# hjurong/hand-pose-estimation

Measured on AMD Instinct MI355X. Metric: particle-evals/sec + tracked FPS, 320x240 depth, 256p x 30gen, higher is better.
Workload: dtype f32+f64

## Files before the change

hand-pose-estimation_amd/csrc/hpe_api.inc:

```
#include <chrono>
#include <cmath>
#include <cstdarg>
#include <cstdlib>
#include <cstdio>
#include <cstring>
#include <new>
#include <string>
#include <thread>
#include <vector>

#include <dlfcn.h>
#include <mutex>

#include <hip/hip_ext.h>
#include <rccl/rccl.h>

#include "../../include/hpe.h"
#include "hpe_host.hpp"

namespace {

#define HPE_RAW_RING 8

struct Slot {
// ... 278 lines not shown
    static constexpr int wpp2_max_p = 1024;
    bool fk_coop = true;
    bool use_graph = true;
    bool prep_split = true;
    double *h_pinned = nullptr;
    int *d_evals = nullptr;
    MwJob *d_mw_job = nullptr;
    double *d_mw_part = nullptr;
    unsigned *d_mw_ctr = nullptr;
    int *d_mw_err = nullptr;
    int *h_mw_err = nullptr, *h_mw_err_dev = nullptr;
    int mw_spin = MW_SPIN_MAX;
    int mw_fits = -1;
    bool refine_mw = true;
    bool refine_exact = false;
    unsigned long long captures = 0;
    int xch_every = 0;
    double *xch_ext = nullptr;
    hpe_exchange_fn xch_fn = nullptr;
    void *xch_user = nullptr;
    struct Subswarm {
        ncclComm_t comm = nullptr;
        double *d_script = nullptr;
        int *d_script_k = nullptr;
        int script_frames = 0;
        bool transport() const { return comm || d_script; }
        int nranks = 0, rank = 0;
        bool on = false;
        double *d_gath = nullptr;
        bool graphs = true;
// ... 615 lines not shown
        return HPE_E_HIP;
    }
    hpe::build_dev_hand(*hand, c->hand);
    if (dalloc(&c->d_hand, 1) != hipSuccess ||
        hipMemcpy(c->d_hand, &c->hand, sizeof(DevHand), hipMemcpyHostToDevice) != hipSuccess ||
        dalloc(&c->d_lane_hands, HPE_BATCH_MAX) != hipSuccess || reset_lane_hands(c) != hipSuccess ||
        dalloc(&c->d_state, 32) != hipSuccess || dalloc(&c->d_evals, 4) != hipSuccess ||
        hipMemset(c->d_evals, 0, 4 * sizeof(int)) != hipSuccess ||
        dalloc(&c->d_obs, HPE_MAX_SLOTS) != hipSuccess || dalloc(&c->d_obs_active, 1) != hipSuccess ||
        dalloc(&c->d_seq_obs, 1) != hipSuccess || dalloc(&c->d_seq_cur, 2) != hipSuccess ||
        dalloc(&c->d_mw_job, 1) != hipSuccess ||
        dalloc(&c->d_mw_part, (size_t)MW_MAX_Q * MW_MAX_NODES) != hipSuccess ||
        dalloc(&c->d_mw_ctr, MW_CTR_WORDS) != hipSuccess ||
        hipMemset(c->d_mw_ctr, 0, MW_CTR_WORDS * sizeof(unsigned)) != hipSuccess ||
        dalloc(&c->d_mw_err, 1) != hipSuccess || hipMemset(c->d_mw_err, 0, sizeof(int)) != hipSuccess ||
        hipHostMalloc((void **)&c->h_pinned, sizeof(double) * 256, 0) != hipSuccess ||
        hipHostMalloc((void **)&c->h_mw_err, sizeof(int), hipHostMallocMapped | hipHostMallocCoherent) != hipSuccess ||
        hipHostGetDevicePointer((void **)&c->h_mw_err_dev, c->h_mw_err, 0) != hipSuccess) {
        hpe_destroy(c);
        return HPE_E_HIP;
    }
    c->slots.resize(1);
    if (const char *pf = std::getenv("HPE_PSO_FORM"))
        c->pso_form = std::strcmp(pf, "block") == 0 ? 1 : std::strcmp(pf, "wave") == 0 ? 2 : 0;
    if (const char *wp = std::getenv("HPE_PSO_WPP")) {
        const int v = std::atoi(wp);
        c->pso_wpp = (v == 1 || v == 2) ? v : 0;
    }
    if (const char *fc = std::getenv("HPE_FK_COOP")) c->fk_coop = std::atoi(fc) != 0;
    if (const char *rm = std::getenv("HPE_REFINE_MW")) c->refine_mw = rm[0] != '0';
    if (const char *re = std::getenv("HPE_REFINE_EXACT")) c->refine_exact = re[0] == '1';
    if (const char *sp = std::getenv("HPE_MW_SPIN")) c->mw_spin = std::max(0, std::atoi(sp));
    if (const char *ps = std::getenv("HPE_PREP_SPLIT")) c->prep_split = ps[0] != '0';
    *c->h_mw_err = 0;
    const char *ng = std::getenv("HPE_NO_GRAPH");
    c->use_graph = !(ng && ng[0] == '1');
    *out = c;
    return HPE_OK;
}

static void drop_graphs(hpe_ctx *c) {
    if (c->stream) (void)hipStreamSynchronize(c->stream);
    for (GraphCache &gc : c->graphs) {
        for (auto &e : gc.entries) (void)hipGraphExecDestroy(e.exec);
        gc.entries.clear();
    }
}
// ... 23 lines not shown
    dfree(c->optl.d_obs);
    dfree(c->d_hand);
    dfree(c->d_lane_hands);
    dfree(c->d_theta);
    dfree(c->d_cost);
    dfree(c->d_terms);
    dfree(c->d_S);
    dfree(c->d_J);
    dfree(c->d_match);
    dfree(c->d_state);
    dfree(c->d_evals);
    dfree(c->d_mw_job);
    dfree(c->d_mw_part);
    dfree(c->d_mw_ctr);
    dfree(c->d_mw_err);
    dfree(c->d_render);
    dfree(c->d_obs);
    dfree(c->d_obs_active);
    dfree(c->d_seq_obs);
    dfree(c->d_seq_cur);
    dfree(c->d_bobs);
    dfree(c->d_bcur);
    dfree(c->d_bevals);
    for (auto &a : c->rb.arena) dfree(a);
    dfree(c->rb.d_obs);
    dfree(c->rb.d_info);
    dfree(c->rb.d_tab);
    dfree(c->rb.d_ctr);
    dfree(c->rb.d_raw);
    dfree(c->rb.d_cur);
// ... 516 lines not shown
#define RF_DYN_LDS (126u * 1024u)
static_assert(RF_DYN_LDS >= RF_STAGE_MAX * (3 * sizeof(double) + sizeof(int32_t)), "staging");

static bool mw_fits(hpe_ctx *c) {
    if (c->mw_fits < 0) {
        int per_cu = 0, cus = 0;
        auto k = c->refine_exact ? k_refine<false, true> : k_refine<false, true, true>;
        if (hipOccupancyMaxActiveBlocksPerMultiprocessor(&per_cu, k, RF_NT, prep_lds_bytes()) != hipSuccess ||
            hipDeviceGetAttribute(&cus, hipDeviceAttributeMultiprocessorCount, c->device) != hipSuccess)
            per_cu = cus = 0;
        c->mw_fits = (long)per_cu * cus >= 1 + MW_MAX_Q + PREP_WG ? 1 : 0;
    }
    return c->mw_fits == 1;
}

static int refine_launch(hpe_ctx *c, const FrameIo &io, int do_refine, const PrepArgs *pa = nullptr,
                         const PrepSplit *split = nullptr, DevPick *pick = nullptr) {
    int rc = ensure_match(c, (size_t)(io.n_max > 0 ? io.n_max : 1));
    if (rc) return rc;
    double *d_x0 = io.state;
    PrepArgs none;
    std::memset(&none, 0, sizeof(none));
    const PrepArgs a = pa ? *pa : none;
    const PrepSplit ps = (pa && split) ? *split : PrepSplit{};
    DevMw mw;
    std::memset(&mw, 0, sizeof(mw));
    const DevPick pk = pick ? *pick : DevPick{};
    if (pick) *pick = DevPick{};
    if (io.n_max <= RF_STAGE_MAX) {
        const dim3 grid(pa ? 1 + PREP_WG : 1);
        launch(c, HPE_PROF_REFINE, c->refine_exact ? k_refine<true> : k_refine<true, false, true>,
               grid, dim3(RF_NT), RF_DYN_LDS, d_x0, io.obs, (const DevHand *)c->d_hand,
               c->d_match, c->d_evals, do_refine, a, mw, pk, ps);
    } else if (c->refine_mw && mw_fits(c)) {
        mw.job = c->d_mw_job;
        mw.part = c->d_mw_part;
        mw.ctr = c->d_mw_ctr;
        mw.err = c->d_mw_err;
        mw.err_host = c->h_mw_err_dev;
        mw.Q = MW_MAX_Q;
        mw.spin = c->mw_spin;
        const dim3 grid(1 + MW_MAX_Q + (pa ? PREP_WG : 0));
        launch(c, HPE_PROF_REFINE,
               c->refine_exact ? k_refine<false, true> : k_refine<false, true, true>, grid,
               dim3(RF_NT), (unsigned)prep_lds_bytes(), d_x0, io.obs, (const DevHand *)c->d_hand,
               c->d_match, c->d_evals, do_refine, a, mw, pk, ps);
    } else {
        const dim3 grid(pa ? 1 + PREP_WG : 1);
        launch(c, HPE_PROF_REFINE, c->refine_exact ? k_refine<false> : k_refine<false, false, true>,
               grid, dim3(RF_NT), RF_DYN_LDS, d_x0,
               io.obs, (const DevHand *)c->d_hand, c->d_match, c->d_evals, do_refine, a,
               mw, pk, ps);
    }
    HIPCHK(c, hipGetLastError());
    return HPE_OK;
}

static int mw_check(hpe_ctx *c) {
    if (!c->d_mw_err) return HPE_OK;
    int err = 0;
    HIPCHK(c, hipMemcpy(&err, c->d_mw_err, sizeof(int), hipMemcpyDeviceToHost));
    if (!err && !(c->h_mw_err && *(volatile int *)c->h_mw_err)) return HPE_OK;
    HIPCHK(c, hipStreamSynchronize(c->stream));
    HIPCHK(c, hipMemset(c->d_mw_ctr, 0, MW_CTR_WORDS * sizeof(unsigned)));
    HIPCHK(c, hipMemset(c->d_mw_err, 0, sizeof(int)));
    if (c->h_mw_err) *(volatile int *)c->h_mw_err = 0;
    return fail(c, HPE_E_HIP, "multi-workgroup refine: a helper hand-off timed out (that "
// ... 208 lines not shown
    }
    if (gathered_out && set) {
        HIPCHK(c, hipSetDevice(c->device));
        HIPCHK(c, hipStreamSynchronize(c->stream));
        HIPCHK(c, hipMemcpy(gathered_out, c->ss.d_gath, sizeof(double) * c->ss.nranks * (HPE_DOF + 1),
                            hipMemcpyDeviceToHost));
    }
    return HPE_OK;
}

int hpe_set_refine_exact(hpe_ctx *c, int exact) {
    if (!c) return HPE_E_ARG;
    if (c->refine_exact != (exact != 0)) {
        c->refine_exact = exact != 0;
        c->mw_fits = -1;
        ++c->epoch;
    }
    return HPE_OK;
}

int hpe_get_refine_exact(const hpe_ctx *c) { return c && c->refine_exact ? 1 : 0; }

int hpe_graph_captures(const hpe_ctx *c, uint64_t *n) {
    if (!c || !n) return HPE_E_ARG;
    *n = c->captures;
    return HPE_OK;
}

int hpe_refine_init_pose(hpe_ctx *c, double x0[26], int32_t *evals_out) {
    if (!c) return HPE_E_ARG;
    if (!x0) return fail(c, HPE_E_ARG, "bad arguments");
    HIPCHK(c, hipSetDevice(c->device));
    DevObs o;
    int rc = need_frame(c, &o);
// ... 1558 lines not shown
```

hand-pose-estimation_amd/csrc/hpe_kernels.hip:

```cpp
#include <vector>

#include "hpe_device.hpp"
#include "hpe_prep.hpp"
#include "hpe_report.hpp"
#include "../../include/hpe.h"

__global__ __launch_bounds__(HPE_NT) void k_build(const double *__restrict__ theta, int P,
                                                  const DevHand *__restrict__ Hg,
                                                  double *__restrict__ S_out,
                                                  double *__restrict__ J_out) {
    __shared__ Smem sm;
    const int i = blockIdx.x, t = threadIdx.x;
    stage_hand<HPE_NT>(sm.hand, Hg);
    const DevHand *__restrict__ H = &sm.hand;
    if (t < HPE_DOF) sm.fk.th[t] = theta[(size_t)i * HPE_DOF + t];
    __syncthreads();
    if (t < 64) fk_wave(sm.fk, H);
    __syncthreads();
    if (t < 3 * HPE_NS) S_out[(size_t)i * 3 * HPE_NS + t] = (&sm.fk.S[0][0])[t];
    if (J_out && t < 63) {
        double v;
        if (t < 3) v = sm.fk.th[3 + t];
        else {
            const int row = t / 3, c = t % 3, k = (row - 1) / 4, jr = 1 + (row - 1) % 4;
// ... 786 lines not shown
            wave_sync();
            if (RIGID) rigid_wave<RG_ROT>(nodes[w], hq, thl);
            else fk_wave(nodes[w], H);
            const double al = wave_sum(align_frozen(nodes[w], cs, H, ms, l, 64));
            if (l == 0) mw.part[h * MW_MAX_NODES + w] = al;
        }
        asm volatile("s_waitcnt vmcnt(0)" ::: "memory");
        __syncthreads();
        if (t == 0) {
            __builtin_amdgcn_fence(__ATOMIC_RELEASE, "agent");
            atomicAdd(&mw.ctr[32 * (1 + h % MW_DONE_SHARDS)], 1u);
        }
    }
}

struct GoldShape {
    int n;
    unsigned long long nb;
    unsigned dn, up;
};
#define GOLD_BALANCED 0
#define GOLD_8 1
#define GOLD_4 2
#define GOLD_OPT8 3
#define GOLD_MIX 4
#ifndef HPE_GOLD_POLICY
#define HPE_GOLD_POLICY GOLD_MIX
#endif
template <int POL>
__device__ __forceinline__ GoldShape gold_shape(int ctx) {
// ... 5 lines not shown
    {8, 0x6043414240212000ull, 0xffff7531u, 0xfffff642u},
    {8, 0x6243414240212000ull, 0xfff7f531u, 0xfffff642u},
    {4, 0x0000000043212000ull, 0xfffffff1u, 0xfffff3f2u},
    {4, 0x0000000060402000ull, 0xfffff321u, 0xffffffffu},
    {4, 0x0000000040212000ull, 0xffffff31u, 0xfffffff2u},
    {8, 0xbf8f674340212000ull, 0xffffff31u, 0xf765f4f2u},
    {8, 0x6043414240212000ull, 0xffff7531u, 0xfffff642u},
    {8, 0x6743414240212000ull, 0xfffff531u, 0xf7fff642u},
    {8, 0xa080604340212000ull, 0xf76f5f31u, 0xfffff4f2u},
    {8, 0x6043414240212000ull, 0xffff7531u, 0xfffff642u},
    {4, 0x0000000040212000ull, 0xffffff31u, 0xfffffff2u},
    };
    return ctx == 0 ? T[3 * POL] : ctx == 1 ? T[3 * POL + 1] : T[3 * POL + 2];
}

template <bool MW = false, int POL = GOLD_BALANCED, bool UPD = false, bool RIGID = false, class CV>
__device__ __forceinline__ double gold_tree(RefineSm &rs, const DevObs &o, const CV &cv,
                                            const DevHand *__restrict__ H,
                                            const int32_t *__restrict__ match, double fk,
                                            double gp, double pl, double gl, int &evals,
                                            double *f_acc, FkX *Xt = nullptr,
                                            MwLeader *ml = nullptr, int *flag = nullptr,
                                            const FrozenPts *fp = nullptr, int rblk = 0,
                                            const double *md2p = nullptr) {
    const int t = threadIdx.x, w = t >> 6, l = t & 63;
    StampClock sc;
    sc.start();
    double A = 0, B = 1e100, alpha = 0.5, tk = 0;
    int it = 0, accepted = -1, ctx = 0;
    bool done = false;
    [[maybe_unused]] unsigned long long path = 0;
    while (!done) {
        const GoldShape sh = gold_shape<POL>(ctx);
        const int nn = sh.n;
        double thl = 0.0;
        if (w < nn) {
            const int nbw = (int)((sh.nb >> (8 * w)) & 0xff), len = nbw >> 5, bits = nbw & 31;
            double ga = A, gb = B, gal = alpha;
            for (int k = 0; k < len; ++k) {
                if ((bits >> k) & 1) gold_up(ga, gb, gal);
                else gold_down(ga, gb, gal);
            }
            thl = rs.x0[l < HPE_DOF ? l : 0] + gal * pl;
            if (l < HPE_DOF) rs.w[w].th[l] = thl;
        }
        eval_nodes<MW, RIGID>(rs, nn, o, cv, H, match, Xt, ml, flag, &thl, fp, rblk, md2p);
        if (MW && ml->failed) break;
        int node = 0;
        accepted = -1;
#pragma unroll
// ... 21 lines not shown
            } else {
                gold_down(A, B, alpha);
                node = (int)((sh.dn >> (4 * node)) & 15u);
                ctx = 1;
            }
        }
        if (!done && it >= 30) done = true;
        done = __builtin_amdgcn_readfirstlane(done ? 1 : 0) != 0;
        ctx = __builtin_amdgcn_readfirstlane(ctx);
        if (UPD && done && t < HPE_DOF) rs.x0[t] = rs.x0[t] - tk * gl;
        if (done && accepted >= 0) {
            for (int q = t; q < (int)(offsetof(FkSm, J) / 8); q += RF_NT)
                ((double *)&rs.base)[q] = ((const double *)&rs.w[accepted])[q];
            if (f_acc) *f_acc = rs.f[accepted];
        }
        __syncthreads();
        REF_TS(rs.ts_n, 4);
        sc.lap(19);
    }
    evals += it;
    if (HPE_STAMPS && blockIdx.x == 0 && t == 0) {
        hpe_stamps[9] += (tk != 0) ? 1 : 0;
        hpe_stamps[30] += (unsigned long long)it;
        hpe_stamps[32 + 9] += 1;
    }
#if HPE_STAMPS
    if (t == 0) {
        const unsigned long long k = atomicAdd(&hpe_gold_log[0], 1ull);
        if (k < HPE_GOLD_LOG)
            hpe_gold_log[1 + k] = path | ((unsigned long long)it << 32) |
                                  ((unsigned long long)(tk != 0) << 40);
    }
#endif
    return tk;
}

template <bool STAGED, bool MW = false, bool RIGID = false>
__global__ __launch_bounds__(RF_NT) void k_refine(double *__restrict__ x0g, const DevObs *__restrict__ og,
                                                  const DevHand *__restrict__ Hg,
                                                  int32_t *__restrict__ match_g,
                                                  int *__restrict__ evals_out, int do_refine,
                                                  PrepArgs pa, DevMw mw, DevPick pk, PrepSplit ps) {
    constexpr bool WIN = false;
    const DevWindow pw{};
#include "hpe_refine_body.inc"
}

enum LaneSrc { LANE_SRC_NONE, LANE_SRC_RAW, LANE_SRC_RING, LANE_SRC_U16 };
#define HPE_ACT_TRACK 1
#define HPE_ACT_PREP 2
__device__ __forceinline__ DevSwarm lane_swarm(DevSwarm sw, size_t stride) {
    const size_t off = stride * blockIdx.y;
    sw.xh = (double *)((char *)sw.xh + off);
    sw.pch = (double *)((char *)sw.pch + off);
    sw.pb = (double *)((char *)sw.pb + off);
    sw.v = (double *)((char *)sw.v + off);
    sw.inbox = (double *)((char *)sw.inbox + off);
    sw.gmin = (unsigned long long *)((char *)sw.gmin + off);
    sw.sig = (Sig *)((char *)sw.sig + off);
    sw.gpos = (double *)((char *)sw.gpos + off);
// ... 145 lines not shown
    const DevHand *__restrict__ const Hg = lane_hand<HANDS>(hands);
    double *__restrict__ const x0g = states + (size_t)HPE_STATE_N * blockIdx.y;
    const DevObs *__restrict__ const og = obs + blockIdx.y;
    int32_t *const match_g = nullptr;
    int *__restrict__ const evals_out = evals_b + HPE_EVALS_N * blockIdx.y;
    const int do_refine = SRC == LANE_SRC_NONE ? 1 : do_refine_arg;
    decltype(lane_prep<SRC>(tab, unit, raw_base, cur, 1)) pa{};
    DevWindow pw{};
    if (SRC != LANE_SRC_NONE && blockIdx.x >= 1) {
        pa = lane_prep<SRC>(tab, unit, raw_base, cur, 1);
        if (WIN) pw = wtab[blockIdx.y];
    }
    const DevMw mw{};
    const DevPick pk{};
    const PrepSplit ps{};
#include "hpe_refine_body.inc"
}
static_assert(PREP_NT == RF_NT, "the preparation workgroups ride in the refine launch");

struct WinPar {
    double margin_xy, margin_z, focal;
    int to_cm, pad;
};
__device__ __forceinline__ double wave_min_f64(double v) {
    for (int off = 32; off > 0; off >>= 1) v = fmin(v, __shfl_xor(v, off));
    return v;
}
__device__ __forceinline__ double wave_max_f64(double v) {
    for (int off = 32; off > 0; off >>= 1) v = fmax(v, __shfl_xor(v, off));
    return v;
// ... 292 lines not shown
```

hand-pose-estimation_amd/csrc/hpe_layout.hpp:

```cpp
#pragma once
#include <stdint.h>

#define HPE_NT 512
#define HPE_NW (HPE_NT / 64)
#define HPE_NS 48
#define HPE_MAX_SLOTS 4096
#define HPE_DOF 26
#define HPE_IMG_H 240
#define HPE_IMG_W 320

enum { ST_NORMAL = 1, ST_RP = 2, ST_RG = 3, ST_LINK = 4, ST_OPT_PERM = 5, ST_OPT_RP = 6,
       ST_OPT_RG = 7, ST_OPT_NORMAL = 8 };

struct DevHand {
    double Fc[5], Fs[5], FLc[5], FLs[5];
    double T10x[5], T10y[5];
    double L[5][4];
    double twc[5], tws[5];
    double radii[HPE_NS];
    double wa[HPE_NS], wb[HPE_NS];
    int32_t dg[HPE_NS], ja[HPE_NS];
};

struct DevObs {
// ... 74 lines not shown
    const double *gath;
    double *hist;
    const int *cur;
    int world;
};

struct DevMw {
    MwJob *job;
    double *part;
    unsigned *ctr;
    int *err;
    int *err_host;
    int Q;
    int spin;
};
```

hand-pose-estimation_amd/csrc/hpe_refine_body.inc:

```
    extern __shared__ __align__(16) unsigned char dyn[];
    const int nhelp = MW ? mw.Q : 0;
    if (MW && blockIdx.x >= 1 && (int)blockIdx.x <= nhelp) {
        if (do_refine) mw_helper<RIGID>(mw, blockIdx.x - 1, og, Hg, match_g);
        return;
    }
    if (blockIdx.x >= 1) {
        const unsigned long long t0 = HPE_STAMPS ? __builtin_amdgcn_s_memtime() : 0;
        prep_workgroup<WIN>(pa, blockIdx.x - 1 - nhelp, dyn, &ps, &pw);
        if (HPE_STAMPS && threadIdx.x == 0) {
            const int k = ((int)blockIdx.x - 1 - nhelp < PREP_BANDS) ? 24 : 25;
            atomicAdd(&hpe_stamps[k], __builtin_amdgcn_s_memtime() - t0);
            atomicAdd(&hpe_stamps[32 + k], 1ull);
        }
        return;
    }
    if (!do_refine) return;
    const DevObs o = *og;
    __shared__ RefineSm rs;
    __shared__ DevHand hs;
    const int t = threadIdx.x, w = t >> 6, l = t & 63;
    stage_hand<RF_NT>(hs, Hg);
    const DevHand *__restrict__ H = &hs;
    using CV = std::conditional_t<STAGED, CloudView, CloudGlobal>;
    CV cv;
    int32_t *match = match_g;
    if (STAGED) {
        double *cx = (double *)dyn, *cy = cx + o.n, *cz = cy + o.n;
        for (int p = t; p < o.n; p += RF_NT) {
            cx[p] = gp(o.cx)[p];
            cy[p] = gp(o.cy)[p];
            cz[p] = gp(o.cz)[p];
        }
        if constexpr (STAGED) cv = CV{cx, cy, cz, o.n};
        match = (int32_t *)(cz + o.n);
    }
    if constexpr (!STAGED) cv = obs_cloud(o);
    if (pk.gath) {
        if (w == 0) {
            const double x = pick_apply(pk.gath, pick_best_row(pk.gath, pk.world, l), l, x0g,
                                        pk.hist, pk.cur);
            if (l < HPE_DOF) rs.x0[l] = x;
        }
    } else if (t < HPE_DOF) {
        rs.x0[t] = x0g[t];
    }
    if (t == 0) rs.ts_n = 0;
    REF_TS(rs.ts_n, 0);
    __shared__ int mwflag;
    MwLeader ml{mw, 0u, false};
    __syncthreads();
    if (RIGID) {
        if (w == 0) {
            const double xl = rs.x0[l < HPE_DOF ? l : 0];
            const double thq = (l == 0) ? -180.0 : (l < 6) ? 0.0 : xl;
            if (l < HPE_DOF) rs.w[0].th[l] = thq;
            wave_sync();
            SphXYZ own;
            fk_wave<true>(rs.w[0], H, &own, &thq);
            if (l < HPE_NS) {
                rs.rg.q[l][0] = own.x;
                rs.rg.q[l][1] = own.y * -1;
                rs.rg.q[l][2] = own.z * -1;
            }
// ... 7 lines not shown
                co += (k < 2 || l < 16) ? v : 0.0;
            }
            co = wave_sum(co);
            if (l == 0) rs.rg.C = co;
        }
        __syncthreads();
    }
    StampClock sc;
    sc.start();
    int evals = 0;
    bool base_valid = false;
    const double e = 1e-5;
    const bool small = !MW && STAGED && o.n >= 1 && o.n <= FP_MAX;
    FrozenPts fpts;
    const double md2_l = depth_off_sq(o, H->radii[l < HPE_NS ? l : HPE_NS - 1]);
    for (int blk = 0; blk < 2; ++blk) {
        const int lo = 3 * blk;
        FkX *Xt = nullptr;
        if (RIGID && blk == 1) {
            if (w == 0) rigid_wave<RG_STORE_P>(rs.w[0], rs.rg, rs.x0[l < HPE_DOF ? l : 0], nullptr, rs.rg.P);
            __syncthreads();
        } else if (blk == 1) {
            if (w == 0) {
                if (l < HPE_DOF) rs.w[0].th[l] = rs.x0[l];
                wave_sync();
                fk_wave_t<FK_STORE_X, true>(rs.w[0], H, &rs.X);
            }
            __syncthreads();
            Xt = &rs.X;
        }
        double tol = 1;
        int cnt = 0, iter = 0;
        while (tol > 1e-6 && iter < 15 && cnt < 1 && !(MW && ml.failed)) {
            if (!base_valid) {
                if (t < HPE_DOF) rs.base.th[t] = rs.x0[t];
                __syncthreads();
                if (w == 0) {
                    if (RIGID) {
                        const double thl = rs.x0[l < HPE_DOF ? l : 0];
                        if (blk) rigid_wave<RG_TRANS>(rs.base, rs.rg, thl);
                        else rigid_wave<RG_ROT>(rs.base, rs.rg, thl);
                    } else if (Xt) {
                        fk_wave_t<FK_TRANSLATE>(rs.base, H, Xt);
                    } else {
                        fk_wave<true>(rs.base, H);
                    }
                }
                __syncthreads();
// ... 29 lines not shown
                double al;
                if (small) {
                    const bool spread = RIGID && HPE_RF_SPREAD;
                    const int f0 = (w < 4 || spread) ? 64 * w : (w >= 6) ? 256 + 128 * (w - 6) : 0;
                    const int cnt = (w < 4 || spread) ? 1 : (w >= 6) ? 2 : 0;
                    al = search_align<RF_NT, true>(rs.base, cv, H, match, load_pt(cv, f0 + l),
                                                   f0 + l, BT_GENS, 64, cnt);
                } else {
                    al = search_align<RF_NT, true>(rs.base, cv, H, match, load_pt(cv, t));
                }
                if (young) __builtin_amdgcn_s_setprio(0);
                double co = (!RIGID && t < 144) ? collide_term(rs.base, t, H) : 0.0;
                const double dep = depth_finish(dgc, o, t < HPE_NS);
                const double tot = wave_sum((al * o.lambda + dep) + co);
                if (l == 0) rs.red[w][0] = tot;
                head();
                __syncthreads();
                if (small) load_frozen_pts(fpts, cv, match, l);
                fk = 0;
#pragma unroll
                for (int k = 0; k < RF_NW; ++k) fk += rs.red[k][0];
                if (RIGID) fk = fk + rs.rg.C;
                REF_TS(rs.ts_n, 2);
                if (w < 6) {
                    double f = RIGID ? frozen_tail<true>(rs.w[w], o, cv, H, match, hd,
                                                         small ? &fpts : nullptr, &md2_l)
                                     : frozen_tail(rs.w[w], o, cv, H, match, hd, small ? &fpts : nullptr);
                    if (RIGID) f = f + rs.rg.C;
                    if (l == 0) rs.fg[w] = f;
                }
                __syncthreads();
            }
            ++evals;
            sc.lap(20);
            evals += 6;
            const double *fg = MW ? rs.f : rs.fg;
            const double g0 = (fg[0] - fg[1]) / (2 * e), g1 = (fg[2] - fg[3]) / (2 * e),
                         g2 = (fg[4] - fg[5]) / (2 * e);
            const int dl = l - lo;
            const double gl = (dl == 0) ? g0 : (dl == 1) ? g1 : (dl == 2) ? g2 : 0.0;
            const double pl = -1 * gl;
            if (MW) __syncthreads();
            REF_TS(rs.ts_n, 3);
            sc.lap(21);
            const double q0 = g0 * (-1 * g0), q1 = g1 * (-1 * g1), q2 = g2 * (-1 * g2);
            const double s0 = g0 * g0, s1 = g1 * g1, s2 = g2 * g2;
            const double gp = (blk == 0) ? (q0 + q2) + q1 : q1 + (q0 + q2);
            const double tk = gold_tree<MW, HPE_GOLD_POLICY, true, RIGID>(
                rs, o, cv, H, match, fk, gp, pl, gl, evals, nullptr, Xt, &ml, &mwflag,
                small ? &fpts : nullptr, blk, &md2_l);
            sc.lap(22);
            if (tk == 0) cnt += 1;
            tol = uniform_f64(sqrt((blk == 0) ? (s0 + s2) + s1 : s1 + (s0 + s2)));
            iter += 1;
            base_valid = true;
            REF_TS(rs.ts_n, 5);
            sc.lap(23);
        }
    }
    if (MW) mw_publish(ml, rs, MW_JOB_EXIT, 0);
    REF_TS(rs.ts_n, 7);
    if (t < HPE_DOF) x0g[t] = (MW && ml.failed) ? __builtin_nan("") : rs.x0[t];
    if (t == 0 && evals_out) {
        *evals_out = evals;
        atomicAdd((unsigned long long *)(evals_out + 2), (unsigned long long)evals);
    }
```

hand-pose-estimation_amd/hpe/__init__.py:

```python
from __future__ import annotations

import ctypes as C
import json
from pathlib import Path

import numpy as np

from . import _lib, report, window
from ._lib import HpeError, ptr

__all__ = ["handmodel", "observedmodel", "costfunc", "PSO", "reference_hand", "scaled_hand",
           "HpeError",
           "gnd_truth_err",
           "Context", "preprocess_depth", "reference_bounds", "X0", "depth_u16_to_mm"]

IMG_H, IMG_W = 240, 320
TB_SPHERES = (2, 2, 2, 2)
FG_SPHERES = (4, 2, 2, 2)
SPACING = (-1.86, -1.86, 0.0, 1.91, 3.84)
CMC = (150.0, 107.5, 89.8, 76.5, 59.6)
X0 = np.array([0, -10, -40, 0, 3, 32, 6, 9, 8, 9, 3, 9, 9, 6, 1, 9, 8, 7, 4, 8, 7, 6, 2,
               7, 7, 7], dtype=np.float64)


# ... 52 lines not shown
            self._h = C.c_void_p()

    def __del__(self):
        try:
            self.close()
        except Exception:
            pass

    @property
    def refine_exact(self) -> bool:
        return bool(self.lib.hpe_get_refine_exact(self.h))

    @refine_exact.setter
    def refine_exact(self, exact: bool):
        self.check(self.lib.hpe_set_refine_exact(self.h, 1 if exact else 0))

    def store_frame(self, slot, depth_cm, dt, cloud, scale, dtmax, K):
        depth_cm = np.ascontiguousarray(depth_cm, dtype=np.float64)
        dt = np.ascontiguousarray(dt, dtype=np.float32)
        cloud = np.ascontiguousarray(cloud, dtype=np.float64).reshape(-1, 3)
        f = _lib.Frame(ptr(depth_cm, C.c_double), ptr(dt, C.c_float), ptr(cloud, C.c_double),
                       len(cloud), float(scale), float(dtmax),
                       (C.c_double * 9)(*np.asarray(K, dtype=np.float64).ravel()))
        self.check(self.lib.hpe_store_frame(self._h, slot, C.byref(f)))

    def select_frame(self, slot):
        self.check(self.lib.hpe_select_frame(self._h, slot))

    def prepare_frame(self, slot, depth_mm, to_cm=True, downsample=True, focal=241.42):
        d = np.ascontiguousarray(depth_mm, dtype=np.float32).reshape(IMG_H, IMG_W)
# ... 607 lines not shown
```

hand-pose-estimation_amd/hpe/_lib.py:

```python
from __future__ import annotations

import ctypes as C
import os
from pathlib import Path

import numpy as np

PKG_DIR = Path(__file__).resolve().parent.parent
LIB_PATH = PKG_DIR / "libhpe.so"

PROF_PSO_GEN, PROF_REFINE, PROF_PSO_INIT, PROF_PSO_FINAL, PROF_PREP = 0, 1, 2, 3, 4
PROF_OPT_DESCENT, PROF_OPT_MOVE, PROF_SWARM_BEST, PROF_EXCHANGE = 5, 6, 7, 8
SUBSWARM_ID_BYTES = 128
BATCH_MAX = 16
BATCH_FORM_AUTO, BATCH_FORM_WAVE = 0, 1
WINDOW_OFF, WINDOW_FIXED, WINDOW_FOLLOW = 0, 1, 2
PACING_LOCKSTEP, PACING_FREE = 0, 1
HPE_OK, HPE_E_ARG, HPE_E_HIP, HPE_E_STATE, HPE_E_NOMEM, HPE_E_NODEVICE = 0, -1, -2, -3, -4, -5

dp = C.POINTER(C.c_double)
fp = C.POINTER(C.c_float)
ip = C.POINTER(C.c_int32)


# ... 85 lines not shown
    "hpe_batch_lost": (C.c_int, [C.c_void_p, C.POINTER(C.c_uint32)]),
    "hpe_lane_joints_dev": (C.c_int, [C.c_void_p, C.c_int, C.c_int, C.c_void_p, C.c_double,
                                      C.c_void_p, C.c_void_p]),
    "hpe_build_spheres":(C.c_int, [C.c_void_p, dp, C.c_int, dp, dp]),
    "hpe_eval_costs": (C.c_int, [C.c_void_p, dp, C.c_int, C.c_int, dp, ip]),
    "hpe_cal_cost2": (C.c_int, [C.c_void_p, dp, ip, C.c_int, dp, dp]),
    "hpe_eval_spheres": (C.c_int, [C.c_void_p, dp, C.c_int, C.c_int, ip, dp]),
    "hpe_set_pso_params": (C.c_int, [C.c_void_p, dp, dp, dp, C.c_double, C.c_double,
                                     C.c_double, C.c_int, C.c_double, C.c_double]),
    "hpe_set_seed": (C.c_int, [C.c_void_p, C.c_uint64]),
    "hpe_pso_evolve": (C.c_int, [C.c_void_p, dp, C.c_int, dp, dp]),
    "hpe_pso_optimise": (C.c_int, [C.c_void_p, dp, C.c_int, dp, dp, dp, C.c_int]),
    "hpe_pso_trace": (C.c_int, [C.c_void_p, dp, ip, ip, C.c_int]),
    "hpe_refine_init_pose": (C.c_int, [C.c_void_p, dp, ip]),
    "hpe_set_refine_exact": (C.c_int, [C.c_void_p, C.c_int]),
    "hpe_graph_captures": (C.c_int, [C.c_void_p, C.POINTER(C.c_uint64)]),
    "hpe_set_exchange": (C.c_int, [C.c_void_p, C.c_int, C.c_void_p, C.c_void_p, C.c_void_p]),
    "hpe_pick_best": (C.c_int, [C.c_void_p, C.c_void_p, C.c_int, C.c_void_p]),
    "hpe_subswarm_unique_id": (C.c_int, [C.c_void_p]),
    "hpe_subswarm_init": (C.c_int, [C.c_void_p, C.c_void_p, C.c_int, C.c_int]),
    "hpe_subswarm_init_scripted": (C.c_int, [C.c_void_p, C.c_int, C.c_int, dp, C.c_int]),
    "hpe_subswarm_enable": (C.c_int, [C.c_void_p, C.c_int]),
    "hpe_subswarm_fini": (C.c_int, [C.c_void_p]),
    "hpe_subswarm_info": (C.c_int, [C.c_void_p, ip, ip, ip, ip, dp]),
    "hpe_get_refine_exact": (C.c_int, [C.c_void_p]),
    "hpe_track_frame": (C.c_int, [C.c_void_p, C.c_int, C.c_int, dp, dp]),
    "hpe_track_frame_dev": (C.c_int, [C.c_void_p, C.c_int, C.c_int, C.c_void_p]),
    "hpe_track_sequence_dev": (C.c_int, [C.c_void_p, C.c_int, C.c_int, C.c_void_p, C.c_int,
                                         C.c_int, C.c_int, C.c_void_p]),
    "hpe_track_batch_dev": (C.c_int, [C.c_void_p, C.c_int, C.c_int, C.c_int, C.c_void_p, ip,
                                      C.c_int, C.c_int, C.c_void_p]),
    "hpe_profile_enable": (C.c_int, [C.c_void_p, C.c_int]),
    "hpe_profile_read": (C.c_int, [C.c_void_p, ip, dp, dp, dp]),
    "hpe_profile_read_kernel": (C.c_int, [C.c_void_p, C.c_int, ip, dp, dp, dp]),
    "hpe_refine_eval_count": (C.c_int, [C.c_void_p, C.POINTER(C.c_uint64), C.c_int]),
    "hpe_render_depth": (C.c_int, [C.c_void_p, dp, C.c_double, fp]),
    "hpe_debug_stamps": (C.c_int, [C.POINTER(C.c_uint64)]),
}

EXCHANGE_FN = C.CFUNCTYPE(C.c_int, C.c_void_p, C.c_void_p, C.c_int)
# ... 38 lines not shown
```

include/hpe.h:

```cpp
#ifndef HPE_H
#define HPE_H

#include <stddef.h>
#include <stdint.h>

#ifdef __cplusplus
extern "C" {
#endif

#define HPE_ABI_VERSION 1

#define HPE_OK 0
#define HPE_E_ARG -1
#define HPE_E_HIP -2
#define HPE_E_STATE -3
#define HPE_E_NOMEM -4
#define HPE_E_NODEVICE -5

typedef struct hpe_ctx hpe_ctx;

typedef struct {
    double geo_cm[20];
    double radii_cm[48];
    double cmc_deg[5];
// ... 69 lines not shown
int hpe_subswarm_init_scripted(hpe_ctx *ctx, int nranks, int rank, const double *script,
                               int frames);

typedef int (*hpe_exchange_fn)(void *user, double *d_ext, int generation);
int hpe_set_exchange(hpe_ctx *ctx, int every, double *d_ext, hpe_exchange_fn fn, void *user);

int hpe_pso_trace(hpe_ctx *ctx, double *gbest, int32_t *count, int32_t *topo, int n);

int hpe_pso_optimise(hpe_ctx *ctx, const double x0[26], int num_p, double bestp[26],
                     double *bestcost_out, double *gbest_trace, int trace_len);

int hpe_refine_init_pose(hpe_ctx *ctx, double x0[26], int32_t *evals_out);

int hpe_set_refine_exact(hpe_ctx *ctx, int exact);
int hpe_get_refine_exact(const hpe_ctx *ctx);

int hpe_track_frame(hpe_ctx *ctx, int num_p, int refine, double x0_inout[26],
                    double *cost_out);

int hpe_track_frame_dev(hpe_ctx *ctx, int num_p, int refine, double *d_state);

#define HPE_SEQ_CHUNK 8
#define HPE_SEQ_MAX_CHUNK 32
int hpe_track_sequence_dev(hpe_ctx *ctx, int num_p, int refine, double *d_state,
                           int first_slot, int n, int frames_per_graph, double *d_hist);

#define HPE_BATCH_MAX 16
int hpe_track_batch_dev(hpe_ctx *ctx, int num_p, int refine, int B, double *d_states,
                        const int32_t *first_slots, int n, int frames_per_graph, double *d_hist);

// ... 111 lines not shown
```

Baseline: 25.48 million.

## Speculatively run refine block 1 on a second workgroup during block 0

Adds a speculative runner workgroup to the staged refine kernel. The main workgroup publishes each block-0 iterate through global atomics. The runner starts block-1 optimisation from that iterate and restarts whenever a newer one arrives. When block 0 converges, the main workgroup commits and takes the runner's block-1 result, so the two coordinate-descent phases overlap instead of running serially. This costs an extra workgroup, spin-polling, and added cross-workgroup synchronisation complexity, with an abort fallback if the runner's result does not arrive in time.

Result: faster. 26.47 million (median of 6 runs) (+3.9%).

```diff
diff --git a/hand-pose-estimation_amd/csrc/hpe_api.inc b/hand-pose-estimation_amd/csrc/hpe_api.inc
--- a/hand-pose-estimation_amd/csrc/hpe_api.inc
+++ b/hand-pose-estimation_amd/csrc/hpe_api.inc
@@ -316,6 +316,11 @@
     int mw_fits = -1;
     bool refine_mw = true;
     bool refine_exact = false;
+    bool refine_spec = true;
+    unsigned long long *d_spec_g = nullptr;
+    unsigned *d_spec_ep = nullptr;
+    int spec_spin = SPEC_SPIN_MAX;
+    int spec_fits = -1;
     unsigned long long captures = 0;
     int xch_every = 0;
     double *xch_ext = nullptr;
@@ -961,6 +966,10 @@
         dalloc(&c->d_mw_ctr, MW_CTR_WORDS) != hipSuccess ||
         hipMemset(c->d_mw_ctr, 0, MW_CTR_WORDS * sizeof(unsigned)) != hipSuccess ||
         dalloc(&c->d_mw_err, 1) != hipSuccess || hipMemset(c->d_mw_err, 0, sizeof(int)) != hipSuccess ||
+        dalloc(&c->d_spec_g, SPEC_GRAN) != hipSuccess ||
+        hipMemset(c->d_spec_g, 0, SPEC_GRAN * sizeof(unsigned long long)) != hipSuccess ||
+        dalloc(&c->d_spec_ep, 64) != hipSuccess ||
+        hipMemset(c->d_spec_ep, 0, 64 * sizeof(unsigned)) != hipSuccess ||
         hipHostMalloc((void **)&c->h_pinned, sizeof(double) * 256, 0) != hipSuccess ||
         hipHostMalloc((void **)&c->h_mw_err, sizeof(int), hipHostMallocMapped | hipHostMallocCoherent) != hipSuccess ||
         hipHostGetDevicePointer((void **)&c->h_mw_err_dev, c->h_mw_err, 0) != hipSuccess) {
@@ -978,6 +987,8 @@
     if (const char *rm = std::getenv("HPE_REFINE_MW")) c->refine_mw = rm[0] != '0';
     if (const char *re = std::getenv("HPE_REFINE_EXACT")) c->refine_exact = re[0] == '1';
     if (const char *sp = std::getenv("HPE_MW_SPIN")) c->mw_spin = std::max(0, std::atoi(sp));
+    if (const char *rs = std::getenv("HPE_REFINE_SPEC")) c->refine_spec = rs[0] != '0';
+    if (const char *ss = std::getenv("HPE_SPEC_SPIN")) c->spec_spin = std::max(0, std::atoi(ss));
     if (const char *ps = std::getenv("HPE_PREP_SPLIT")) c->prep_split = ps[0] != '0';
     *c->h_mw_err = 0;
     const char *ng = std::getenv("HPE_NO_GRAPH");
@@ -1031,6 +1042,8 @@
     dfree(c->d_mw_part);
     dfree(c->d_mw_ctr);
     dfree(c->d_mw_err);
+    dfree(c->d_spec_g);
+    dfree(c->d_spec_ep);
     dfree(c->d_render);
     dfree(c->d_obs);
     dfree(c->d_obs_active);
@@ -1577,6 +1590,18 @@
     return c->mw_fits == 1;
 }
 
+static bool spec_fits(hpe_ctx *c) {
+    if (c->spec_fits < 0) {
+        int per_cu = 0, cus = 0;
+        auto k = c->refine_exact ? k_refine<true, false, false, true> : k_refine<true, false, true, true>;
+        if (hipOccupancyMaxActiveBlocksPerMultiprocessor(&per_cu, k, RF_NT, RF_DYN_LDS) != hipSuccess ||
+            hipDeviceGetAttribute(&cus, hipDeviceAttributeMultiprocessorCount, c->device) != hipSuccess)
+            per_cu = cus = 0;
+        c->spec_fits = (long)per_cu * cus >= 2 + PREP_WG ? 1 : 0;
+    }
+    return c->spec_fits == 1;
+}
+
 static int refine_launch(hpe_ctx *c, const FrameIo &io, int do_refine, const PrepArgs *pa = nullptr,
                          const PrepSplit *split = nullptr, DevPick *pick = nullptr) {
     int rc = ensure_match(c, (size_t)(io.n_max > 0 ? io.n_max : 1));
@@ -1590,11 +1615,19 @@
     std::memset(&mw, 0, sizeof(mw));
     const DevPick pk = pick ? *pick : DevPick{};
     if (pick) *pick = DevPick{};
-    if (io.n_max <= RF_STAGE_MAX) {
+    const DevSpec nosp{};
+    if (io.n_max <= RF_STAGE_MAX && c->refine_spec && spec_fits(c)) {
+        const DevSpec sp{c->d_spec_g, c->d_spec_ep, c->spec_spin};
+        const dim3 grid(pa ? 2 + PREP_WG : 2);
+        launch(c, HPE_PROF_REFINE,
+               c->refine_exact ? k_refine<true, false, false, true> : k_refine<true, false, true, true>,
+               grid, dim3(RF_NT), RF_DYN_LDS, d_x0, io.obs, (const DevHand *)c->d_hand,
+               c->d_match, c->d_evals, do_refine, a, mw, pk, ps, sp);
+    } else if (io.n_max <= RF_STAGE_MAX) {
         const dim3 grid(pa ? 1 + PREP_WG : 1);
         launch(c, HPE_PROF_REFINE, c->refine_exact ? k_refine<true> : k_refine<true, false, true>,
                grid, dim3(RF_NT), RF_DYN_LDS, d_x0, io.obs, (const DevHand *)c->d_hand,
-               c->d_match, c->d_evals, do_refine, a, mw, pk, ps);
+               c->d_match, c->d_evals, do_refine, a, mw, pk, ps, nosp);
     } else if (c->refine_mw && mw_fits(c)) {
         mw.job = c->d_mw_job;
         mw.part = c->d_mw_part;
@@ -1607,13 +1640,13 @@
         launch(c, HPE_PROF_REFINE,
                c->refine_exact ? k_refine<false, true> : k_refine<false, true, true>, grid,
                dim3(RF_NT), (unsigned)prep_lds_bytes(), d_x0, io.obs, (const DevHand *)c->d_hand,
-               c->d_match, c->d_evals, do_refine, a, mw, pk, ps);
+               c->d_match, c->d_evals, do_refine, a, mw, pk, ps, nosp);
     } else {
         const dim3 grid(pa ? 1 + PREP_WG : 1);
         launch(c, HPE_PROF_REFINE, c->refine_exact ? k_refine<false> : k_refine<false, false, true>,
                grid, dim3(RF_NT), RF_DYN_LDS, d_x0,
                io.obs, (const DevHand *)c->d_hand, c->d_match, c->d_evals, do_refine, a,
-               mw, pk, ps);
+               mw, pk, ps, nosp);
     }
     HIPCHK(c, hipGetLastError());
     return HPE_OK;
@@ -1852,10 +1885,22 @@
     if (c->refine_exact != (exact != 0)) {
         c->refine_exact = exact != 0;
         c->mw_fits = -1;
+        c->spec_fits = -1;
         ++c->epoch;
     }
     return HPE_OK;
 }
+
+int hpe_set_refine_spec(hpe_ctx *c, int on) {
+    if (!c) return HPE_E_ARG;
+    if (c->refine_spec != (on != 0)) {
+        c->refine_spec = on != 0;
+        ++c->epoch;
+    }
+    return HPE_OK;
+}
+
+int hpe_get_refine_spec(const hpe_ctx *c) { return c && c->refine_spec ? 1 : 0; }
 
 int hpe_get_refine_exact(const hpe_ctx *c) { return c && c->refine_exact ? 1 : 0; }
 
diff --git a/hand-pose-estimation_amd/csrc/hpe_kernels.hip b/hand-pose-estimation_amd/csrc/hpe_kernels.hip
--- a/hand-pose-estimation_amd/csrc/hpe_kernels.hip
+++ b/hand-pose-estimation_amd/csrc/hpe_kernels.hip
@@ -824,6 +824,112 @@
     }
 }
 
+#define SPEC_SPIN_MAX 1024
+#define SPEC_IDLE_SPIN (1 << 20)
+#define SPEC_PW (RF_NW - 1)
+
+struct SpecSm {
+    unsigned half[SPEC_X0_GRAN];
+    int verdict;
+    int evals;
+    double res[3];
+};
+struct SpecPoll {
+    DevSpec sp;
+    SpecSm *sm;
+    unsigned ep;
+    int seq;
+};
+
+__device__ __forceinline__ unsigned long long spec_load(const unsigned long long *p) {
+    return __hip_atomic_load(p, __ATOMIC_RELAXED, __HIP_MEMORY_SCOPE_AGENT);
+}
+__device__ __forceinline__ void spec_store(unsigned long long *p, unsigned tag, unsigned v) {
+    __hip_atomic_store(p, ((unsigned long long)tag << 32) | v, __ATOMIC_RELAXED, __HIP_MEMORY_SCOPE_AGENT);
+}
+__device__ __forceinline__ unsigned spec_half(double x, int hi) {
+    const unsigned long long b = (unsigned long long)__double_as_longlong(x);
+    return hi ? (unsigned)(b >> 32) : (unsigned)b;
+}
+__device__ __forceinline__ void spec_send(const DevSpec &sp, unsigned tag, const double *x0) {
+    const int l = threadIdx.x & 63;
+    if (l < SPEC_X0_GRAN) spec_store(sp.g + l, tag, spec_half(x0[l >> 1], l & 1));
+}
+__device__ __forceinline__ unsigned long long spec_poll_issue(const DevSpec &sp) {
+    const int l = threadIdx.x & 63;
+    return spec_load(sp.g + (l < SPEC_CTL ? l : SPEC_CTL));
+}
+__device__ __forceinline__ int spec_poll_take(SpecSm &sm, unsigned long long g, unsigned ep,
+                                              int seq, int *commit = nullptr) {
+    const int l = threadIdx.x & 63;
+    const unsigned tag = (unsigned)(g >> 32), val = (unsigned)g;
+    const unsigned t0 = (unsigned)__builtin_amdgcn_readlane((int)tag, 0);
+    const unsigned ct = (unsigned)__builtin_amdgcn_readlane((int)tag, SPEC_CTL);
+    const unsigned cv = (unsigned)__builtin_amdgcn_readlane((int)val, SPEC_CTL);
+    const bool whole = __all(l >= SPEC_X0_GRAN || tag == t0) != 0;
+    const bool mine = (ct >> 5) == ep;
+    int v = 0;
+    if (mine && cv == SPEC_ABORT) {
+        v = -1;
+    } else if (whole && (t0 >> 5) == ep && (int)(t0 & 31u) > seq) {
+        v = (int)(t0 & 31u);
+        if (l < SPEC_X0_GRAN) sm.half[l] = val;
+    }
+    if (commit) *commit = (mine && cv == SPEC_COMMIT) ? (int)(ct & 31u) : 0;
+    if (l == 0) sm.verdict = v;
+    return v;
+}
+__device__ __forceinline__ int spec_wait(const DevSpec &sp, SpecSm &sm, unsigned ep, int seq, bool done) {
+    __syncthreads();
+    if (threadIdx.x < 64) {
+        int v = -1;
+        for (int i = 0; i < SPEC_IDLE_SPIN; ++i) {
+            int commit = 0;
+            const int r = spec_poll_take(sm, spec_poll_issue(sp), ep, seq, &commit);
+            if (r != 0 || (done && commit == seq)) {
+                v = r;
+                break;
+            }
+            __builtin_amdgcn_s_sleep(2);
+        }
+        if (threadIdx.x == 0) sm.verdict = v;
+    }
+    __syncthreads();
+    return __builtin_amdgcn_readfirstlane(sm.verdict);
+}
+__device__ __forceinline__ void spec_take_x0(const SpecSm &sm, double *x0) {
+    const int t = threadIdx.x;
+    if (t < HPE_DOF)
+        x0[t] = __longlong_as_double((long long)(((unsigned long long)sm.half[2 * t + 1] << 32) | sm.half[2 * t]));
+    __syncthreads();
+}
+__device__ __forceinline__ void spec_result(const DevSpec &sp, unsigned tag, const double *x0, int evals) {
+    const int l = threadIdx.x & 63;
+    if (l < 6) spec_store(sp.g + SPEC_RES + l, tag, spec_half(x0[3 + (l >> 1)], l & 1));
+    else if (l == 6) spec_store(sp.g + SPEC_RES + 6, tag, (unsigned)evals);
+}
+__device__ __forceinline__ bool spec_commit(const DevSpec &sp, SpecSm &sm, unsigned tag, bool failed) {
+    const int l = threadIdx.x & 63;
+    bool ok = false;
+    if (failed && sp.spin > 0) {
+        if (l == 0) spec_store(sp.g + SPEC_CTL, tag, SPEC_COMMIT);
+        for (int i = 0; i < sp.spin && !ok; ++i) {
+            const unsigned long long g = spec_load(sp.g + SPEC_RES + (l < 7 ? l : 6));
+            ok = __all((unsigned)(g >> 32) == tag) != 0;
+            if (ok) {
+                const unsigned lo = (unsigned)__shfl((int)(unsigned)g, (l << 1) & 63);
+                const unsigned hi = (unsigned)__shfl((int)(unsigned)g, ((l << 1) + 1) & 63);
+                if (l < 3) sm.res[l] = __longlong_as_double((long long)(((unsigned long long)hi << 32) | lo));
+                if (l == 6) sm.evals = (int)(unsigned)g;
+            } else {
+                __builtin_amdgcn_s_sleep(2);
+            }
+        }
+    }
+    if (!ok && l == 0) spec_store(sp.g + SPEC_CTL, tag, SPEC_ABORT);
+    return ok;
+}
+
 struct GoldShape {
     int n;
     unsigned long long nb;
@@ -859,7 +965,8 @@
     return ctx == 0 ? T[3 * POL] : ctx == 1 ? T[3 * POL + 1] : T[3 * POL + 2];
 }
 
-template <bool MW = false, int POL = GOLD_BALANCED, bool UPD = false, bool RIGID = false, class CV>
+template <bool MW = false, int POL = GOLD_BALANCED, bool UPD = false, bool RIGID = false,
+          bool POLL = false, class CV>
 __device__ __forceinline__ double gold_tree(RefineSm &rs, const DevObs &o, const CV &cv,
                                             const DevHand *__restrict__ H,
                                             const int32_t *__restrict__ match, double fk,
@@ -867,7 +974,8 @@
                                             double *f_acc, FkX *Xt = nullptr,
                                             MwLeader *ml = nullptr, int *flag = nullptr,
                                             const FrozenPts *fp = nullptr, int rblk = 0,
-                                            const double *md2p = nullptr) {
+                                            const double *md2p = nullptr,
+                                            const SpecPoll *poll = nullptr, int *drop = nullptr) {
     const int t = threadIdx.x, w = t >> 6, l = t & 63;
     StampClock sc;
     sc.start();
@@ -879,6 +987,8 @@
         const GoldShape sh = gold_shape<POL>(ctx);
         const int nn = sh.n;
         double thl = 0.0;
+        [[maybe_unused]] unsigned long long pg = 0;
+        if constexpr (POLL) if (w == SPEC_PW) pg = spec_poll_issue(poll->sp);
         if (w < nn) {
             const int nbw = (int)((sh.nb >> (8 * w)) & 0xff), len = nbw >> 5, bits = nbw & 31;
             double ga = A, gb = B, gal = alpha;
@@ -930,7 +1040,15 @@
                 ((double *)&rs.base)[q] = ((const double *)&rs.w[accepted])[q];
             if (f_acc) *f_acc = rs.f[accepted];
         }
+        if constexpr (POLL) if (w == SPEC_PW) spec_poll_take(*poll->sm, pg, poll->ep, poll->seq);
         __syncthreads();
+        if constexpr (POLL) {
+            const int v = __builtin_amdgcn_readfirstlane(poll->sm->verdict);
+            if (v != 0) {
+                *drop = v;
+                break;
+            }
+        }
         REF_TS(rs.ts_n, 4);
         sc.lap(19);
     }
@@ -941,7 +1059,7 @@
         hpe_stamps[32 + 9] += 1;
     }
 #if HPE_STAMPS
-    if (t == 0) {
+    if (t == 0 && !POLL) {
         const unsigned long long k = atomicAdd(&hpe_gold_log[0], 1ull);
         if (k < HPE_GOLD_LOG)
             hpe_gold_log[1 + k] = path | ((unsigned long long)it << 32) |
@@ -951,15 +1069,36 @@
     return tk;
 }
 
-template <bool STAGED, bool MW = false, bool RIGID = false>
+template <bool STAGED, bool MW = false, bool RIGID = false, bool SPEC = false>
 __global__ __launch_bounds__(RF_NT) void k_refine(double *__restrict__ x0g, const DevObs *__restrict__ og,
                                                   const DevHand *__restrict__ Hg,
                                                   int32_t *__restrict__ match_g,
                                                   int *__restrict__ evals_out, int do_refine,
-                                                  PrepArgs pa, DevMw mw, DevPick pk, PrepSplit ps) {
+                                                  PrepArgs pa, DevMw mw, DevPick pk, PrepSplit ps,
+                                                  DevSpec sp) {
+    static_assert(!SPEC || (STAGED && !MW), "the runner stages the cloud; no helpers");
     constexpr bool WIN = false;
     const DevWindow pw{};
+    if constexpr (!SPEC) {
+        constexpr bool RUNNER = false;
+        SpecSm *const ssm_p = nullptr;
 #include "hpe_refine_body.inc"
+    } else {
+        extern __shared__ __align__(16) unsigned char dyn[];
+        __shared__ RefineSm rs;
+        __shared__ DevHand hs;
+        __shared__ int mwflag;
+        __shared__ SpecSm ssm;
+        SpecSm *const ssm_p = &ssm;
+        auto body = [&](auto role) {
+            constexpr bool RUNNER = decltype(role)::value;
+#define HPE_REFINE_BODY_NO_DECLS
+#include "hpe_refine_body.inc"
+#undef HPE_REFINE_BODY_NO_DECLS
+        };
+        if (blockIdx.x == 1) body(std::true_type{});
+        else body(std::false_type{});
+    }
 }
 
 enum LaneSrc { LANE_SRC_NONE, LANE_SRC_RAW, LANE_SRC_RING, LANE_SRC_U16 };
@@ -1135,6 +1274,9 @@
     const DevMw mw{};
     const DevPick pk{};
     const PrepSplit ps{};
+    constexpr bool SPEC = false, RUNNER = false;
+    const DevSpec sp{};
+    SpecSm *const ssm_p = nullptr;
 #include "hpe_refine_body.inc"
 }
 static_assert(PREP_NT == RF_NT, "the preparation workgroups ride in the refine launch");
diff --git a/hand-pose-estimation_amd/csrc/hpe_layout.hpp b/hand-pose-estimation_amd/csrc/hpe_layout.hpp
--- a/hand-pose-estimation_amd/csrc/hpe_layout.hpp
+++ b/hand-pose-estimation_amd/csrc/hpe_layout.hpp
@@ -112,3 +112,15 @@
     int Q;
     int spin;
 };
+
+#define SPEC_X0_GRAN (2 * HPE_DOF)
+#define SPEC_CTL SPEC_X0_GRAN
+#define SPEC_RES 64
+#define SPEC_GRAN 96
+#define SPEC_EP_MASK 0x7ffffffu
+enum { SPEC_COMMIT = 1, SPEC_ABORT = 2 };
+struct DevSpec {
+    unsigned long long *g;
+    unsigned *epoch;
+    int spin;
+};
diff --git a/hand-pose-estimation_amd/csrc/hpe_refine_body.inc b/hand-pose-estimation_amd/csrc/hpe_refine_body.inc
--- a/hand-pose-estimation_amd/csrc/hpe_refine_body.inc
+++ b/hand-pose-estimation_amd/csrc/hpe_refine_body.inc
@@ -1,10 +1,13 @@
+#ifndef HPE_REFINE_BODY_NO_DECLS
     extern __shared__ __align__(16) unsigned char dyn[];
-    const int nhelp = MW ? mw.Q : 0;
+#endif
+    const int nhelp = MW ? mw.Q : SPEC ? 1 : 0;
+    constexpr bool runner = SPEC && RUNNER;
     if (MW && blockIdx.x >= 1 && (int)blockIdx.x <= nhelp) {
         if (do_refine) mw_helper<RIGID>(mw, blockIdx.x - 1, og, Hg, match_g);
         return;
     }
-    if (blockIdx.x >= 1) {
+    if (blockIdx.x >= 1 && !runner) {
         const unsigned long long t0 = HPE_STAMPS ? __builtin_amdgcn_s_memtime() : 0;
         prep_workgroup<WIN>(pa, blockIdx.x - 1 - nhelp, dyn, &ps, &pw);
         if (HPE_STAMPS && threadIdx.x == 0) {
@@ -15,9 +18,15 @@
         return;
     }
     if (!do_refine) return;
+    unsigned sp_ep = 0;
+    if constexpr (SPEC)
+        sp_ep = (__hip_atomic_load(sp.epoch + (runner ? 32 : 0), __ATOMIC_RELAXED, __HIP_MEMORY_SCOPE_AGENT) + 1u) &
+                SPEC_EP_MASK;
     const DevObs o = *og;
+#ifndef HPE_REFINE_BODY_NO_DECLS
     __shared__ RefineSm rs;
     __shared__ DevHand hs;
+#endif
     const int t = threadIdx.x, w = t >> 6, l = t & 63;
     stage_hand<RF_NT>(hs, Hg);
     const DevHand *__restrict__ H = &hs;
@@ -35,7 +44,16 @@
         match = (int32_t *)(cz + o.n);
     }
     if constexpr (!STAGED) cv = obs_cloud(o);
-    if (pk.gath) {
+    [[maybe_unused]] int sp_seq = 0;
+    if constexpr (runner) {
+        sp_seq = spec_wait(sp, *ssm_p, sp_ep, 0, false);
+        if (sp_seq <= 0) {
+            if (t == 0)
+                __hip_atomic_store(sp.epoch + 32, sp_ep, __ATOMIC_RELAXED, __HIP_MEMORY_SCOPE_AGENT);
+            return;
+        }
+        spec_take_x0(*ssm_p, rs.x0);
+    } else if (pk.gath) {
         if (w == 0) {
             const double x = pick_apply(pk.gath, pick_best_row(pk.gath, pk.world, l), l, x0g,
                                         pk.hist, pk.cur);
@@ -46,7 +64,9 @@
     }
     if (t == 0) rs.ts_n = 0;
     REF_TS(rs.ts_n, 0);
+#ifndef HPE_REFINE_BODY_NO_DECLS
     __shared__ int mwflag;
+#endif
     MwLeader ml{mw, 0u, false};
     __syncthreads();
     if (RIGID) {
@@ -84,7 +104,12 @@
     const bool small = !MW && STAGED && o.n >= 1 && o.n <= FP_MAX;
     FrozenPts fpts;
     const double md2_l = depth_off_sq(o, H->radii[l < HPE_NS ? l : HPE_NS - 1]);
-    for (int blk = 0; blk < 2; ++blk) {
+    [[maybe_unused]] int verdict = 0;
+    [[maybe_unused]] SpecPoll spoll{};
+spec_again:
+    __attribute__((unused));
+    if constexpr (runner) spoll = SpecPoll{sp, ssm_p, sp_ep, sp_seq};
+    for (int blk = runner ? 1 : 0; blk < 2; ++blk) {
         const int lo = 3 * blk;
         FkX *Xt = nullptr;
         if (RIGID && blk == 1) {
@@ -102,6 +127,10 @@
         double tol = 1;
         int cnt = 0, iter = 0;
         while (tol > 1e-6 && iter < 15 && cnt < 1 && !(MW && ml.failed)) {
+            if constexpr (SPEC && !runner) if (blk == 0) {
+                sp_seq += 1;
+                if (w == SPEC_PW) spec_send(sp, (sp_ep << 5) | (unsigned)sp_seq, rs.x0);
+            }
             if (!base_valid) {
                 if (t < HPE_DOF) rs.base.th[t] = rs.x0[t];
                 __syncthreads();
@@ -161,6 +190,8 @@
                 const double dep = depth_finish(dgc, o, t < HPE_NS);
                 const double tot = wave_sum((al * o.lambda + dep) + co);
                 if (l == 0) rs.red[w][0] = tot;
+                [[maybe_unused]] unsigned long long pg = 0;
+                if constexpr (runner) if (w == SPEC_PW) pg = spec_poll_issue(sp);
                 head();
                 __syncthreads();
                 if (small) load_frozen_pts(fpts, cv, match, l);
@@ -176,7 +207,12 @@
                     if (RIGID) f = f + rs.rg.C;
                     if (l == 0) rs.fg[w] = f;
                 }
-                __syncthreads();
+                if constexpr (runner) if (w == SPEC_PW) spec_poll_take(*ssm_p, pg, sp_ep, sp_seq);
+                __syncthreads();
+                if constexpr (runner) {
+                    verdict = __builtin_amdgcn_readfirstlane(ssm_p->verdict);
+                    if (verdict != 0) break;
+                }
             }
             ++evals;
             sc.lap(20);
@@ -193,9 +229,10 @@
             const double q0 = g0 * (-1 * g0), q1 = g1 * (-1 * g1), q2 = g2 * (-1 * g2);
             const double s0 = g0 * g0, s1 = g1 * g1, s2 = g2 * g2;
             const double gp = (blk == 0) ? (q0 + q2) + q1 : q1 + (q0 + q2);
-            const double tk = gold_tree<MW, HPE_GOLD_POLICY, true, RIGID>(
+            const double tk = gold_tree<MW, HPE_GOLD_POLICY, true, RIGID, runner>(
                 rs, o, cv, H, match, fk, gp, pl, gl, evals, nullptr, Xt, &ml, &mwflag,
-                small ? &fpts : nullptr, blk, &md2_l);
+                small ? &fpts : nullptr, blk, &md2_l, &spoll, &verdict);
+            if constexpr (runner) if (verdict != 0) break;
             sc.lap(22);
             if (tk == 0) cnt += 1;
             tol = uniform_f64(sqrt((blk == 0) ? (s0 + s2) + s1 : s1 + (s0 + s2)));
@@ -204,7 +241,40 @@
             REF_TS(rs.ts_n, 5);
             sc.lap(23);
         }
-    }
+        if constexpr (SPEC && !runner) if (blk == 0) {
+            REF_TS(rs.ts_n, 6);
+            if (w == 0) {
+                const bool ok = spec_commit(sp, *ssm_p, (sp_ep << 5) | (unsigned)sp_seq, cnt >= 1);
+                if (l == 0) ssm_p->verdict = ok ? 1 : 0;
+            }
+            __syncthreads();
+            if (__builtin_amdgcn_readfirstlane(ssm_p->verdict)) {
+                if (t < 3) rs.x0[3 + t] = ssm_p->res[t];
+                evals += __builtin_amdgcn_readfirstlane(ssm_p->evals);
+                __syncthreads();
+                break;
+            }
+        }
+    }
+    if constexpr (runner) {
+        if (verdict == 0) verdict = spec_wait(sp, *ssm_p, sp_ep, sp_seq, true);
+        if (verdict > 0) {
+            __syncthreads();
+            spec_take_x0(*ssm_p, rs.x0);
+            sp_seq = verdict;
+            verdict = 0;
+            evals = 0;
+            base_valid = false;
+            goto spec_again;
+        }
+        if (verdict == 0 && w == 0)
+            spec_result(sp, (sp_ep << 5) | (unsigned)sp_seq, rs.x0, evals);
+    }
+    if constexpr (SPEC) {
+        if (t == 0)
+            __hip_atomic_store(sp.epoch + (runner ? 32 : 0), sp_ep, __ATOMIC_RELAXED, __HIP_MEMORY_SCOPE_AGENT);
+    }
+    if constexpr (runner) return;
     if (MW) mw_publish(ml, rs, MW_JOB_EXIT, 0);
     REF_TS(rs.ts_n, 7);
     if (t < HPE_DOF) x0g[t] = (MW && ml.failed) ? __builtin_nan("") : rs.x0[t];
diff --git a/hand-pose-estimation_amd/hpe/__init__.py b/hand-pose-estimation_amd/hpe/__init__.py
--- a/hand-pose-estimation_amd/hpe/__init__.py
+++ b/hand-pose-estimation_amd/hpe/__init__.py
@@ -90,6 +90,14 @@
     @refine_exact.setter
     def refine_exact(self, exact: bool):
         self.check(self.lib.hpe_set_refine_exact(self.h, 1 if exact else 0))
+
+    @property
+    def refine_spec(self) -> bool:
+        return bool(self.lib.hpe_get_refine_spec(self.h))
+
+    @refine_spec.setter
+    def refine_spec(self, on: bool):
+        self.check(self.lib.hpe_set_refine_spec(self.h, 1 if on else 0))
 
     def store_frame(self, slot, depth_cm, dt, cloud, scale, dtmax, K):
         depth_cm = np.ascontiguousarray(depth_cm, dtype=np.float64)
diff --git a/hand-pose-estimation_amd/hpe/_lib.py b/hand-pose-estimation_amd/hpe/_lib.py
--- a/hand-pose-estimation_amd/hpe/_lib.py
+++ b/hand-pose-estimation_amd/hpe/_lib.py
@@ -123,6 +123,7 @@
     "hpe_pso_trace": (C.c_int, [C.c_void_p, dp, ip, ip, C.c_int]),
     "hpe_refine_init_pose": (C.c_int, [C.c_void_p, dp, ip]),
     "hpe_set_refine_exact": (C.c_int, [C.c_void_p, C.c_int]),
+    "hpe_set_refine_spec": (C.c_int, [C.c_void_p, C.c_int]),
     "hpe_graph_captures": (C.c_int, [C.c_void_p, C.POINTER(C.c_uint64)]),
     "hpe_set_exchange": (C.c_int, [C.c_void_p, C.c_int, C.c_void_p, C.c_void_p, C.c_void_p]),
     "hpe_pick_best": (C.c_int, [C.c_void_p, C.c_void_p, C.c_int, C.c_void_p]),
@@ -133,6 +134,7 @@
     "hpe_subswarm_fini": (C.c_int, [C.c_void_p]),
     "hpe_subswarm_info": (C.c_int, [C.c_void_p, ip, ip, ip, ip, dp]),
     "hpe_get_refine_exact": (C.c_int, [C.c_void_p]),
+    "hpe_get_refine_spec": (C.c_int, [C.c_void_p]),
     "hpe_track_frame": (C.c_int, [C.c_void_p, C.c_int, C.c_int, dp, dp]),
     "hpe_track_frame_dev": (C.c_int, [C.c_void_p, C.c_int, C.c_int, C.c_void_p]),
     "hpe_track_sequence_dev": (C.c_int, [C.c_void_p, C.c_int, C.c_int, C.c_void_p, C.c_int,
diff --git a/include/hpe.h b/include/hpe.h
--- a/include/hpe.h
+++ b/include/hpe.h
@@ -107,6 +107,9 @@
 
 int hpe_set_refine_exact(hpe_ctx *ctx, int exact);
 int hpe_get_refine_exact(const hpe_ctx *ctx);
+
+int hpe_set_refine_spec(hpe_ctx *ctx, int on);
+int hpe_get_refine_spec(const hpe_ctx *ctx);
 
 int hpe_track_frame(hpe_ctx *ctx, int num_p, int refine, double x0_inout[26],
                     double *cost_out);
```
